# ricklisz/AnatoMask

Hardware: AMD Instinct MI355X
Metric: pretrain volumes/sec @128^3 patch mask=0.6 (higher is better)
Workload: dtype bf16; 1 GPU; STUNet-B AnatoMask step, 128^3 patch, mask_ratio 0.6, bf16 storage/MFMA + fp32 master; per_gpu_batch=16, global_batch=16, parallelism=dp1, step=teacher fwd + sampler + student fwd + loss + bwd + clip + AdamW + EMA

## Files before the change

### anatomask_amd/csrc/conv_igemm.hip

```cpp
#include <mutex>
#include <type_traits>
#include <stdlib.h>
#include "common.h"
#include "../../include/anatomask_hip.h"
#include "conv_plan.h"

using namespace amconv;

namespace {

template <typename T, int BD, int BH, int BW, int NS, int NIT, int TGS = 3, bool HR = false, bool NB = false, bool HT = false>
__global__ __launch_bounds__(256, (TGS == 2 && BD * BH * BW <= 256) ? 3 : 2) void conv_igemm_kernel(ConvArgs a) {
  constexpr int EPC = TT<T>::EPC;
  constexpr bool SPL = std::is_same<T, f32s_t>::value;
  constexpr int KC = (ROWB / 16) * EPC;
  constexpr int MV = BD * BH * BW;
  constexpr int VS = MV / 64;
  constexpr int NT = 16 * NS;
  constexpr int TG = TG_OF(NS, TGS);
  constexpr int WBUF = TG * NT * ROWB;
  constexpr int WCH = TG * NT * 4;
  constexpr int WIT = (WCH + 255) / 256;
  static_assert(MV % 64 == 0, "brick must give each wave whole 16-voxel subtiles");
  extern __shared__ __attribute__((aligned(16))) unsigned char lds[];
// ... 592 lines not shown
  p.in_sparse = p.out_sparse = sparse; p.same_mask = p.has_list = true;
  p.in_bshift = in_bshift; p.out_bshift = out_bshift; p.n_active = n_active;
}

extern "C" int am_conv3d_partials_rows(int mode, int dtype, int ksize, int stride, int B, int Do, int Ho, int Wo, int Cin, int Cout, int out_sparse,
                                       int out_bshift, int n_active, int* rows) {
  ConvProblem p{mode, dtype, ksize, stride, B, Do, Ho, Wo, Cin, Do, Ho, Wo, Cout};
  query_masks(p, out_sparse != 0, out_bshift, out_bshift, n_active);
  *rows = 0;
  for (const ConvStage& s : conv_stages) { const int r = s.fits(p); if (r > *rows) *rows = r; }
  return 0;
}

extern "C" int am_conv3d_uses_k3(int mode, int dtype, int ksize, int stride, int B, int Di, int Hi, int Wi, int Cin, int Do, int Ho, int Wo, int Cout,
                                 int has_masks, int accumulate, int fused_epilogue, int want_partials) {
  ConvProblem p{mode, dtype, ksize, stride, B, Di, Hi, Wi, Cin, Do, Ho, Wo, Cout};
  query_masks(p, has_masks != 0, 0, 0, 0);
  p.accumulate = accumulate != 0; p.ep = fused_epilogue != 0; p.partials = want_partials != 0;
  for (const ConvStage& s : conv_stages)
    if (s.serves(p)) return s.launch == conv_k3t_launch ? 2 : s.launch == conv_k3_launch ? 1 : 0;
  return 0;
}

static ConvArgs fill_args(const ConvProblem& p, const void* x, const void* w_packed, const float* bias, void* y, float* partials, const uint8_t* in_mask,
                          int in_bshift, const uint8_t* out_mask, int out_bshift, int fd, int fh, int fw, int accumulate) {
  ConvArgs a{};
  a.x = x; a.w = w_packed; a.bias = bias; a.y = y; a.partials = partials;
  a.B = p.B; a.Di = p.Di; a.Hi = p.Hi; a.Wi = p.Wi; a.Cin = p.Cin; a.Do = p.Do; a.Ho = p.Ho; a.Wo = p.Wo; a.Cout = p.Cout;
  am_packed_dims(p.dtype, p.Cout, p.Cin, &a.Coutp, &a.Cinp);
  a.w_bytes = p.ksize * p.ksize * p.ksize * a.Coutp * a.Cinp * (p.dtype == AM_DT_BF16 ? 2 : 4);
  a.in_mask = MaskView{in_mask, fd, fh, fw, in_bshift};
  a.out_mask = MaskView{out_mask, fd, fh, fw, out_bshift};
  a.accumulate = accumulate & 1; a.stats_sum_only = (accumulate & AM_CONV_PARTIALS_SUM_ONLY) ? 1 : 0;
#ifdef AM_ABLATE
  { const char* e = getenv("AM_CV_DBG"); a.dbg = e ? atoi(e) : 0; }
#endif
  return a;
}

static int conv3d_impl(ConvProblem& p, ConvArgs& a, const int* active_list, int n_active, void* stream, int* rows) {
  if (p.Cin % 8 || p.Cout % 8) return -1;
  p.in_sparse = a.in_mask.m != nullptr; p.out_sparse = a.out_mask.m != nullptr; p.same_mask = a.in_mask.m == a.out_mask.m;
  p.in_bshift = a.in_mask.bs; p.out_bshift = a.out_mask.bs; p.fd = a.in_mask.fd; p.fh = a.in_mask.fh; p.fw = a.in_mask.fw;
  p.has_list = active_list != nullptr; p.n_active = n_active;
  p.accumulate = a.accumulate != 0; p.sum_only = a.stats_sum_only != 0; p.partials = a.partials != nullptr;
  p.ep = a.ep_scale || a.ep_res || a.ep_act != AM_ACT_NONE; p.nbred = a.nb_x != nullptr; p.prenorm = a.in_scale != nullptr;
// ... 24 lines not shown
  query_masks(p, true, in_bshift, out_bshift, n_active);
  p.prenorm = true;
  return conv_rw_serves(p) ? 1 : 0;
}

extern "C" int am_conv3d_prenorm(int mode, int dtype, int ksize, int stride, const void* x, const void* w_packed, const float* bias, void* y,
                                 int B, int Di, int Hi, int Wi, int Cin, int Do, int Ho, int Wo, int Cout, const uint8_t* mask, int in_bshift,
                                 int out_bshift, int fd, int fh, int fw, float* partials, const float* in_scale, const float* in_shift,
                                 int in_act, const int32_t* active_list, int n_active, int* partial_rows_written, void* stream) {
  if (!in_scale || !in_shift || !mask || !active_list) return -1;
  if (in_act != AM_ACT_NONE && in_act != AM_ACT_LRELU && in_act != AM_ACT_RELU6) return -1;
  ConvProblem p{mode, dtype, ksize, stride, B, Di, Hi, Wi, Cin, Do, Ho, Wo, Cout};
  ConvArgs a = fill_args(p, x, w_packed, bias, y, partials, mask, in_bshift, mask, out_bshift, fd, fh, fw, 0);
  a.in_scale = in_scale; a.in_shift = in_shift; a.in_act = in_act;
  return conv3d_impl(p, a, active_list, n_active, stream, partial_rows_written);
}

extern "C" int am_conv3d_nbred(int mode, int dtype, int ksize, int stride, const void* x, const void* w_packed, void* y, int B, int Di,
                               int Hi, int Wi, int Cin, int Do, int Ho, int Wo, int Cout, const uint8_t* in_mask, int in_bshift,
                               const uint8_t* out_mask, int out_bshift, int fd, int fh, int fw, int accumulate, float* partials,
                               const void* nb_x, const float* nb_scale, const float* nb_shift, int nb_act,
                               int* partial_rows_written, void* stream) {
  if (dtype != AM_DT_BF16 || !partials || !nb_x) return -1;
  if (nb_act != AM_ACT_NONE && (!nb_scale || !nb_shift)) return -1;
  if (nb_act != AM_ACT_NONE && nb_act != AM_ACT_LRELU && nb_act != AM_ACT_RELU6) return -1;
  ConvProblem p{mode, dtype, ksize, stride, B, Di, Hi, Wi, Cin, Do, Ho, Wo, Cout};
  ConvArgs a = fill_args(p, x, w_packed, nullptr, y, partials, in_mask, in_bshift, out_mask, out_bshift, fd, fh, fw, accumulate);
  a.nb_x = nb_x; a.nb_scale = nb_scale; a.nb_shift = nb_shift; a.nb_act = nb_act;
  return conv3d_impl(p, a, nullptr, 0, stream, partial_rows_written);
}
```

### anatomask_amd/csrc/conv_k3.hip

```cpp
#include <stdlib.h>
#include "common.h"
#include "../../include/anatomask_hip.h"
#include "conv_plan.h"

using namespace amconv;

namespace {

constexpr int KBD = 8, KBH = 4, KBW = 16;
constexpr int KED = KBD + 2, KEH = KBH + 2, KEW = KBW + 2;
constexpr int KPLANE = KEH * KEW;
constexpr int KNROW = KED * KPLANE;
constexpr int KBRICKB = KNROW * 64;
constexpr int KNPIECE = 68;
constexpr int KWSLOT = 3 * 64 * 64;
constexpr int KLDS_W = 2 * KBRICKB;
constexpr int KLDS_TAB = KLDS_W + 2 * KWSLOT;
constexpr int KLDS = KLDS_TAB + 768;
#ifndef AM_K3_MIN_UNITS
#define AM_K3_MIN_UNITS 256
#endif
constexpr int K3_MIN_UNITS = AM_K3_MIN_UNITS;

struct K3Args {
// ... 5 lines not shown
  int nt_store;
  unsigned w_bytes;
#ifdef AM_ABLATE
  int dbg;
#endif
};

#define K3_LDSP(off) ((__attribute__((address_space(3))) void*)(lds + (off)))

__device__ __forceinline__ int k3_uni(int v) { return __builtin_amdgcn_readfirstlane(v); }
template <typename P> __device__ __forceinline__ P* k3_uni_ptr(P* p) {
  const unsigned long long v = (unsigned long long)p;
  const unsigned lo = (unsigned)__builtin_amdgcn_readfirstlane((int)(unsigned)v), hi = (unsigned)__builtin_amdgcn_readfirstlane((int)(unsigned)(v >> 32));
  return (P*)(((unsigned long long)hi << 32) | lo);
}

struct Item { int u, k, c0, c1, p; };
#define IT_Q0W(it) (((it).c0 & 255) * KBW)
#define IT_Q0H(it) ((((it).c0 >> 8) & 255) * KBH)
#define IT_Q0D(it) ((((it).c0 >> 16) & 255) * KBD)
#define IT_B(it) ((it).c1 & 255)
#define IT_CO0(it) (((it).c1 >> 8) * NT)

template <int NS, bool EP, bool ST, bool CT = false, bool S1 = false>
__global__ __launch_bounds__(512, 2) void conv_k3_kernel(K3Args a) {
  static_assert(NS == 4 || NS == 2, "64- or 32-channel output tiles (NS = 2: the decoder's last conv, C -> C / 2 = 32 at STUNet-B; a wave then owns 8 accumulator tiles)");
  constexpr int VS = 4, NT = 16 * NS;
  constexpr int NCH = VS * NS / 2;
  constexpr int NRUN = CT ? 4 : 9;
  constexpr int NTR = CT ? 2 : 3;
  static_assert(!CT || (NS == 4 && !EP && !ST), "transposed conv: 64-channel tiles, plain epilogue (bias)");
  static_assert(!S1 || (ST && NS == 4 && !CT), "sum-only statistics: a variant of the statistics instantiation");
  extern __shared__ __attribute__((aligned(16))) unsigned char lds[];
  const int tid = threadIdx.x, lane = tid & 63;
  const int wave = __builtin_amdgcn_readfirstlane(tid >> 6);
  const bool isX = wave < 4;
  const int wq = wave & 3;
  const int g = lane >> 4, r16 = lane & 15;
  const int G = gridDim.x;

  const int gperm = (G % 8 == 0) ? (int)(blockIdx.x % 8) * (G / 8) + (int)(blockIdx.x / 8) : (int)blockIdx.x;
  auto decode = [&](Item& it) {
    int br = it.u / a.ny;
    const int yt = it.u - br * a.ny;
    const int bw_ = br % a.nbw; br /= a.nbw;
    const int bh_ = br % a.nbh; br /= a.nbh;
    const int bd_ = br % a.nbd;
    it.c0 = k3_uni(bw_ | (bh_ << 8) | (bd_ << 16)); it.c1 = k3_uni((br / a.nbd) | (yt << 8));
  };
  auto advance = [&](Item& it) {
    if (it.k + 1 < a.nslab) { ++it.k; return; }
    it.k = 0;
    if (CT && it.p < 7) { ++it.p; return; }
    it.p = 0; it.u += G;
    if (it.u < a.nunit) decode(it);
// ... 48 lines not shown
    const long long org = ((((long long)IT_B(it) * a.D + (q0d - 1)) * a.H + (q0h - 1)) * a.W + (q0w - 1)) * (long long)a.Cin;
    const __amdgpu_buffer_rsrc_t rx = __builtin_amdgcn_make_buffer_rsrc((void*)k3_uni_ptr(a.x + org), 0, 0x7fffff00, 0x00020000);
#pragma unroll
    for (int k = k0; k < k1; ++k) {
      const unsigned bad = pbits[k / 5] & (m << (6 * (k % 5)));
      unsigned vo = bad ? OOB : pl[k];
#ifdef AM_ABLATE
      if (a.dbg & 2) vo = OOB;
#endif
      const int p = wave + 8 * k;
      const int row0 = p * 16 < KNROW - 16 ? p * 16 : KNROW - 16;
      __builtin_amdgcn_raw_ptr_buffer_load_lds(rx, K3_LDSP(sbuf * KBRICKB + row0 * 64), 16, vo, (unsigned)(it.k * 64), 0, 0);
    }
  };

  f32x4 acc[NS][VS];
  float f1[NS / 2][4], f2[NS / 2][4];
#pragma unroll
  for (int h = 0; h < NS / 2; ++h)
#pragma unroll
    for (int r = 0; r < 4; ++r) { f1[h][r] = 0.f; f2[h][r] = 0.f; }
  const unsigned oddm = (lane & 1) ? 0xffffffffu : 0u;
#ifdef AM_ABLATE
  const bool want_stats = ST && a.partials != nullptr && !(a.dbg & 32);
#else
  const bool want_stats = ST && a.partials != nullptr;
#endif
  bf16_t* __restrict__ yg = a.y;
  const float act_slope = a.ep_act == AM_ACT_LRELU ? 0.01f : (a.ep_act == AM_ACT_RELU6 ? 0.f : 1.f);
  const float act_hi = a.ep_act == AM_ACT_RELU6 ? 6.f : __builtin_inff();
  constexpr bool fused = EP;
  typedef __attribute__((ext_vector_type(4))) __bf16 bfx4;
  typedef __attribute__((ext_vector_type(8))) __bf16 bfx8;
  typedef __attribute__((ext_vector_type(8))) float f32x8;

  auto flush_stats = [&](const int co0) __attribute__((always_inline)) {
    float* part = a.partials + ((size_t)blockIdx.x * 8 + wave) * a.Cout * 2;
#define K3_DPP_ADD(V, CTRL) V += __builtin_bit_cast(float, __builtin_amdgcn_update_dpp(0, __builtin_bit_cast(int, V), CTRL, 0xF, 0xF, true))
#pragma unroll
    for (int h = 0; h < NS / 2; ++h)
#pragma unroll
      for (int r = 0; r < 4; ++r) {
        float s1 = f1[h][r], s2 = f2[h][r];
        K3_DPP_ADD(s1, 0x4E); K3_DPP_ADD(s1, 0x124); K3_DPP_ADD(s1, 0x128);
        if constexpr (!S1) { K3_DPP_ADD(s2, 0x4E); K3_DPP_ADD(s2, 0x124); K3_DPP_ADD(s2, 0x128); }
        const int c = co0 + h * 32 + g * 8 + (r16 & 1) * 4 + r;
        if (r16 < 2) { part[c * 2] = s1; part[c * 2 + 1] = s2; }
      }
#undef K3_DPP_ADD
// ... 86 lines not shown
  auto store_chunk = [&](const int c, const bool tail) __attribute__((always_inline)) {
    const int j = c / (NS / 2), h = c % (NS / 2);
    const __amdgpu_buffer_rsrc_t ry = __builtin_amdgcn_make_buffer_rsrc((void*)k3_uni_ptr(yg + pk_off), 0, 0x7fffff00, 0x00020000);
#ifdef AM_ABLATE
    if (!(a.dbg & 1))
#endif
    {
      u32x4 sv = pk[j][h];
      unsigned so_ = (unsigned)(j * orow + h * 64);
      if constexpr (FULL) {
        const u32x4 ot = pk[j][h ^ 1];
        u32x4 rx_;
#pragma unroll
        for (int e = 0; e < 4; ++e) rx_[e] = (unsigned)__builtin_amdgcn_update_dpp(0, (int)ot[e], 0x128, 0xF, 0xF, false);
        const bool own = h == 0 ? lo8 : !lo8;
#pragma unroll
        for (int e = 0; e < 4; ++e) sv[e] = own ? sv[e] : rx_[e];
        so_ = (unsigned)(j * orow) + (h ? ohalf : 0u);
      }
      if (a.nt_store) __builtin_amdgcn_raw_buffer_store_b128(sv, ry, olane, so_, 2);
      else __builtin_amdgcn_raw_buffer_store_b128(sv, ry, olane, so_, 0);
      if (tail || FULL) asm volatile("s_nop 4" : "+v"(sv) :: "memory");
    }
    if (want_stats && (tail || !spread_stats)) { stats_half(c, 0); stats_half(c, 1); }
  };

  if (want_stats && a.ny > 1) {
    float* part = a.partials + ((size_t)blockIdx.x * 8 + wave) * a.Cout * 2;
    for (int c = lane; c < a.Cout * 2; c += 64) part[c] = 0.f;
    asm volatile("s_waitcnt vmcnt(0)" ::: "memory");
  }
  if (tid < NT) {
    const int c = IT_CO0(cur) + tid;
    ((float*)(lds + KLDS_TAB))[tid] = a.bias ? a.bias[c] : 0.f;
    ((float*)(lds + KLDS_TAB))[64 + tid] = a.ep_scale ? a.ep_scale[c] : 1.f;
    ((float*)(lds + KLDS_TAB))[128 + tid] = a.ep_scale ? a.ep_shift[c] : 0.f;
  }
  if (isX) { issue_weights(cur, 0, 0); issue_pieces(cur, 0, 0, 9); }
  else issue_pieces(cur, 0, 0, 8);
  asm volatile("s_waitcnt vmcnt(0) lgkmcnt(0)" ::: "memory");
  __builtin_amdgcn_s_barrier();

#ifdef AM_ABLATE
  unsigned tL = 0, tWL = 0, tM = 0, tWM = 0, tE = 0, t_prev = 0;
  unsigned long long rt0 = 0;
  const bool stamps = (a.dbg & 16) != 0;
#define K3_STAMP(ACC) if (stamps) { unsigned long long t_; asm volatile("s_memtime %0\n\ts_waitcnt lgkmcnt(0)" : "=s"(t_) :: "memory"); ACC += (unsigned)t_ - t_prev; t_prev = (unsigned)t_; }
// ... 5 lines not shown
  int pc0 = 0, pc1 = 0, pcls = 0; bool have_prev = false;
  bool spend = false;
  bool pend_stats = false;
#pragma unroll
  for (int i = 0; i < NS; ++i)
#pragma unroll
    for (int j = 0; j < VS; ++j) acc[i][j] = f32x4{0.f, 0.f, 0.f, 0.f};
  while (true) {
    spend = false;
    if (cur.k == 0 && have_prev) {
      finish_unit(pc0, pc1, pcls);
      spend = true; pend_stats = true;
      K3_STAMP(tE);
    } else if (cur.k >= 2) pend_stats = false;
    const bool has_next = nxt.u < a.nunit;
    int bxc[3];
#pragma unroll
    for (int xw = 0; xw < 3; ++xw) bxc[xw] = bx[xw] + sb * KBRICKB;
    const bool fetch_next = has_next && (!CT || a.nslab != 2 || nxt.p == 0);
    const int cpd = (cur.p >> 2) & 1, cph = (cur.p >> 1) & 1, cpw = cur.p & 1;
#pragma unroll
    for (int run = 0; run < NRUN; ++run) {
      const int zd = run / 3, xw = run % 3;
      u32x4 brow[VS + 2], af[3][NS];
      const int wbase = KLDS_W + par * KWSLOT + aoff;
      if constexpr (CT) {
        const int zq = cpd + (run >> 1), xq = cpw + (run & 1);
        const int bsel = (xq == 0 ? bxc[0] : (xq == 1 ? bxc[1] : bxc[2])) + (zq * KPLANE + cph * KEW) * 64;
#pragma unroll
        for (int r = 0; r < VS + 1; ++r) brow[r] = *(const u32x4*)(lds + bsel + r * KEW * 64);
      } else {
#pragma unroll
      for (int r = 0; r < VS + 2; ++r) brow[r] = *(const u32x4*)(lds + bxc[xw] + (zd * KPLANE + r * KEW) * 64);
      }
#pragma unroll
      for (int th = 0; th < NTR; ++th)
#pragma unroll
        for (int i = 0; i < NS; ++i) af[th][i] = *(const u32x4*)(lds + wbase + th * (NT * 64) + i * 1024);
      const int pk0 = CT ? (isX ? 3 * run : 4 * run) : (run == 0 ? 0 : (run == 1 ? 1 : run + 1));
      const int npx = CT ? (run < 3 ? 3 : 0) : (run == 1 ? 2 : (run < 8 ? 1 : 0));
      const int npy = CT ? (run < 2 ? 4 : 0) : (run == 1 ? 2 : (run < 7 ? 1 : 0));
      constexpr int SPR = CT ? 2 : 1;
      if (isX) {
        if (run < NRUN - 1) issue_weights(cur, run + 1, par ^ 1);
        else if (has_next) issue_weights(nxt, 0, par ^ 1);
        if (fetch_next && npx > 0) issue_pieces(nxt, sb ^ 1, CT ? 3 * run : pk0, (CT ? 3 * run : pk0) + npx);
// ... 38 lines not shown
        else if (nbehind == 2) asm volatile("s_waitcnt vmcnt(2)" ::: "memory");
        else if (nbehind == 3) asm volatile("s_waitcnt vmcnt(3)" ::: "memory");
        else if (nbehind == 4) asm volatile("s_waitcnt vmcnt(4)" ::: "memory");
        else asm volatile("s_waitcnt vmcnt(5)" ::: "memory");
      } else if (run == NRUN - 2) {
        if (spend && run * SPR < NCH) { if (SPR == 2) asm volatile("s_waitcnt vmcnt(2)" ::: "memory"); else asm volatile("s_waitcnt vmcnt(1)" ::: "memory"); }
        else asm volatile("s_waitcnt vmcnt(0)" ::: "memory");
      }
      K3_STAMP(tM);
      if (isX) {
        __builtin_amdgcn_s_barrier();
        K3_STAMP(tWM);
      }
      par ^= 1;
    }
    sb ^= 1;
    if (cur.k + 1 == a.nslab) { pc0 = cur.c0; pc1 = cur.c1; pcls = cur.p; have_prev = true; }
    if (!has_next) break;
    cur = nxt; advance(nxt);
  }
  finish_unit(pc0, pc1, pcls);
#pragma unroll
  for (int c = 0; c < NCH; ++c) store_chunk(c, true);
  if (want_stats) flush_stats((pc1 >> 8) * NT);
#ifdef AM_ABLATE
  if (stamps && a.partials) {
    K3_STAMP(tE);
    unsigned long long rt1; asm volatile("s_memrealtime %0\n\ts_waitcnt lgkmcnt(0)" : "=s"(rt1) :: "memory");
    unsigned* row = (unsigned*)(a.partials + ((size_t)blockIdx.x * 8 + wave) * a.Cout * 2);
    asm volatile("s_waitcnt vmcnt(0)" ::: "memory");
    if (lane == 0) { row[0] = tL; row[1] = tWL; row[2] = tM; row[3] = tWM; row[4] = tE; row[5] = (unsigned)(rt1 - rt0); }
  }
#endif
}

}

namespace amconv {

static int k3_tiles(int Cout) { return Cout % 64 ? Cout / 32 : Cout / 64; }
static int k3_units(int B, int D, int H, int W, int Cout) { return B * (D / KBD) * (H / KBH) * (W / KBW) * k3_tiles(Cout); }
static int k3_grid(int units, int Cout, int dev = am_device()) {
  const int cus = am_cu_count(dev), ny = k3_tiles(Cout);
  const int G = units < cus ? units : cus;
  return G - G % ny > 0 ? G - G % ny : ny;
}

static bool k3_qualifies(int mode, int dtype, int ksize, int stride, int B, int D, int H, int W, int Cin, int Cout, bool masks) {
  if (dtype != AM_DT_BF16 || ksize != 3 || stride != 1 || (mode != AM_CONV_FWD && mode != AM_CONV_DGRAD) || masks) return false;
  if (Cin % 32 || Cout % 32 || D % KBD || H % KBH || W % KBW) return false;
  if (B > 255 || D / KBD > 255 || H / KBH > 255 || W / KBW > 255) return false;
  return k3_units(B, D, H, W, Cout) >= K3_MIN_UNITS;
}

int conv_k3_fits(const ConvProblem& p) {
  if (!k3_qualifies(p.mode, p.dtype, p.ksize, p.stride, p.B, p.Do, p.Ho, p.Wo, p.Cin, p.Cout, p.in_sparse || p.out_sparse)) return 0;
  return k3_grid(k3_units(p.B, p.Do, p.Ho, p.Wo, p.Cout), p.Cout) * 8;
}

bool conv_k3_serves(const ConvProblem& p) {
#ifdef AM_ABLATE
  if (getenv("AM_CV_NORW") || getenv("AM_CV_NOK3")) return false;
  { const char* e_ = getenv("AM_K3_NO32"); if (e_ && atoi(e_) && p.Cout % 64) return false; }
#endif
  if (!conv_k3_fits(p) || p.prenorm || p.accumulate || p.nbred) return false;
  if (p.Di != p.Do || p.Hi != p.Ho || p.Wi != p.Wo) return false;
  if ((size_t)(KED + 1) * p.Hi * p.Wi * p.Cin * 2 >= 0x7fffff00ull) return false;
  if (p.ep && p.partials) return false;
  return true;
}

int conv_k3t_fits(const ConvProblem&) { return 0; }
bool conv_k3t_serves(const ConvProblem& p) {
#ifdef AM_ABLATE
  if (getenv("AM_CV_NORW")) return false;
  { const char* e_ = getenv("AM_CV_NOK3T"); if (e_ && atoi(e_)) return false; }
#endif
  if (p.mode != AM_CONVT_FWD || p.dtype != AM_DT_BF16 || p.ksize != 4 || p.stride != 2 || p.in_sparse || p.out_sparse) return false;
  if (p.prenorm || p.accumulate || p.nbred || p.partials || p.ep) return false;
  if (p.Cin % 32 || p.Cin < 64 || p.Cout % 64 || p.Di % KBD || p.Hi % KBH || p.Wi % KBW) return false;
  if (p.Do != 2 * p.Di || p.Ho != 2 * p.Hi || p.Wo != 2 * p.Wi) return false;
  if (p.B > 255 || p.Di / KBD > 255 || p.Hi / KBH > 255 || p.Wi / KBW > 255) return false;
  if ((size_t)(KED + 1) * p.Hi * p.Wi * p.Cin * 2 >= 0x7fffff00ull || (size_t)16 * p.Wo * p.Cout * 2 >= 0x7fffff00ull) return false;
  return k3_units(p.B, p.Di, p.Hi, p.Wi, p.Cout) >= K3_MIN_UNITS;
}

static void k3_fill(K3Args& a, const ConvProblem& p, const ConvArgs& c) {
  a.x = (const bf16_t*)c.x; a.w = (const bf16_t*)c.w; a.bias = c.bias; a.y = (bf16_t*)c.y; a.partials = c.partials;
  a.ep_scale = c.ep_scale; a.ep_shift = c.ep_shift; a.ep_res = (const bf16_t*)c.ep_res; a.ep_act = c.ep_act;
  a.B = c.B; a.D = c.Di; a.H = c.Hi; a.W = c.Wi; a.Cin = c.Cin; a.Cout = c.Cout; a.Cinp = c.Cinp; a.Coutp = c.Coutp;
  a.nbd = c.Di / KBD; a.nbh = c.Hi / KBH; a.nbw = c.Wi / KBW; a.ny = k3_tiles(c.Cout); a.nunit = k3_units(c.B, c.Di, c.Hi, c.Wi, c.Cout); a.nslab = c.Cinp / 32;
  a.flip = p.mode == AM_CONV_DGRAD;
  a.nt_store = (size_t)c.B * c.Do * c.Ho * c.Wo * c.Cout * 2 >= ((size_t)384 << 20);
  a.w_bytes = (unsigned)c.w_bytes;
#ifdef AM_ABLATE
  { const char* e = getenv("AM_K3_DBG"); a.dbg = e ? atoi(e) : 0; }
#endif
}

int conv_k3_launch(const ConvProblem& p, ConvArgs& c, const int*, void* stream, int* rows) {
  if (!conv_k3_serves(p)) return 0;
  const int dev = am_device();
  K3Args a;
  k3_fill(a, p, c);
  const int G = k3_grid(a.nunit, c.Cout, dev);
  auto kern = p.ep ? conv_k3_kernel<4, true, false> : (a.partials ? conv_k3_kernel<4, false, true> : conv_k3_kernel<4, false, false>);
  if (c.Cout % 64) kern = p.ep ? conv_k3_kernel<2, true, false> : (a.partials ? conv_k3_kernel<2, false, true> : conv_k3_kernel<2, false, false>);
  else if (a.partials && !p.ep && c.stats_sum_only) kern = conv_k3_kernel<4, false, true, false, true>;
  AM_HIP_STAGE((am_lds_optin<conv_k3_kernel<4, true, false>, conv_k3_kernel<4, false, true>, conv_k3_kernel<4, false, false>,
                             conv_k3_kernel<2, true, false>, conv_k3_kernel<2, false, true>, conv_k3_kernel<2, false, false>,
                             conv_k3_kernel<4, false, true, false, true>>(dev)));
  AM_LAUNCH(kern, dim3(G), dim3(512), KLDS, (hipStream_t)stream, a);
  AM_CHECK_LAUNCH_STAGE();
  if (rows) *rows = G * 8;
  return 1;
}

int conv_k3t_launch(const ConvProblem& p, ConvArgs& c, const int*, void* stream, int*) {
  if (!conv_k3t_serves(p)) return 0;
  const int dev = am_device();
  K3Args a;
  k3_fill(a, p, c);
  constexpr auto kern = conv_k3_kernel<4, false, false, true>;
  AM_HIP_STAGE(am_lds_optin<kern>(dev));
  AM_LAUNCH(kern, dim3(k3_grid(a.nunit, c.Cout, dev)), dim3(512), KLDS, (hipStream_t)stream, a);
  AM_CHECK_LAUNCH_STAGE();
  return 1;
}

}
```

### anatomask_amd/csrc/conv_plan.h

```cpp
#pragma once
#include "common.h"

namespace amconv {

struct ConvArgs {
  const void* x; const void* w; const float* bias; void* y; float* partials;
  const float* ep_scale; const float* ep_shift; const void* ep_res; int ep_act;
  const void* nb_x; const float* nb_scale; const float* nb_shift; int nb_act;
  const float* in_scale; const float* in_shift; int in_act;
  int B, Di, Hi, Wi, Cin, Do, Ho, Wo, Cout, Cinp, Coutp;
  int OS, GS, nclass, nunit;
  int ny;
  int nbd, nbh, nbw;
  int tap_begin[9];
  int upar[8];
  int taps[64];
  int mind[8], minh[8], minw[8];
  int ed[8], eh[8], ew[8];
  int mdiv_w[8], mdiv_hw[8];
  int w_bytes;
  int w_lds_off;
  MaskView in_mask, out_mask;
  int accumulate;
  int stats_sum_only;
// ... 81 lines not shown
  return 0;
}


struct ConvProblem {
  int mode, dtype, ksize, stride, B, Di, Hi, Wi, Cin, Do, Ho, Wo, Cout;
  bool in_sparse, out_sparse, same_mask, has_list;
  int in_bshift, out_bshift, n_active, fd, fh, fw;
  bool accumulate, ep, partials, sum_only;
  bool nbred, prenorm;
};

struct ConvStage {
  const char* name;
  int (*fits)(const ConvProblem&);
  bool (*serves)(const ConvProblem&);
  int (*launch)(const ConvProblem&, ConvArgs& a, const int* active_list, void* stream, int* rows);
};
#define AM_CONV_STAGE(name_) int name_##_fits(const ConvProblem&); bool name_##_serves(const ConvProblem&); \
                             int name_##_launch(const ConvProblem&, ConvArgs&, const int*, void*, int*)
AM_CONV_STAGE(conv_k3t); AM_CONV_STAGE(conv_k3);
AM_CONV_STAGE(conv_rw); AM_CONV_STAGE(conv_gather);
AM_CONV_STAGE(conv_igemm);

}
```

### anatomask_amd/engine.py

```python
from __future__ import annotations

from dataclasses import dataclass, field
from typing import Dict, List, Optional, Sequence, Tuple

import torch

from . import ops
from .ops import ACT_LRELU, ACT_NONE, ACT_RELU6, CONV_DGRAD, CONV_FWD, CONVT_DGRAD, CONVT_FWD, MaskInfo, NormStats

ENC = "sparse_encoder.sp_cnn.conv_blocks_context"
DEC = "dense_decoder.dec"


@dataclass
class Spec:
    dims: Sequence[int]
    depth: Sequence[int]
    width: int
    input_size: Tuple[int, int, int]
    in_ch: int = 1
    out_ch: int = 1
    downsample: int = 16
    n_stage: int = 5
    sync_bn: bool = False
# ... 392 lines not shown
    def run():
        dwp = ops.conv3d_wgrad(mode, x, dy, k, stride, f32_split=pk.f32_split, deterministic=pk.deterministic, **masks)
        ops.unpack_grad(dwp, G[name], transposed, accumulate=True)
    _on_side(x.device, (x, dy), run)


def _dec_block_backward(W, G, pk: PackCache, t: dict, g: Optional[torch.Tensor], drec: Optional[torch.Tensor], bias_sum_into: Optional[torch.Tensor]):
    q = t["q"]
    if t.get("inorm"):
        so = tuple(t["r"].shape[1:4])
        dc2 = _instance_norm_backward(g, t["c2"], t["st2"], ACT_NONE)
        dr = ops.conv3d(CONV_DGRAD, dc2, pk.get(W, f"{q}.conv.3.weight", False, True), None, so, 3, 1)
        _wgrad_into(pk, G, f"{q}.conv.3.weight", CONV_FWD, t["r"], dc2, 3, 1)
        dc1 = _instance_norm_backward(dr, t["c1"], t["st1"], ACT_RELU6)
    elif t.get("head"):
        dc2 = ops.proj_norm_bwd(t["c2"], t["st2"], drec, W["dense_decoder.proj.weight"].view(-1), W[f"{q}.conv.4.weight"],
                                W[f"{q}.conv.4.bias"], G[f"{q}.conv.4.weight"], G[f"{q}.conv.4.bias"],
                                G["dense_decoder.proj.weight"].view(-1), G["dense_decoder.proj.bias"])
    else:
        dc2 = ops.norm_backward(g, None, t["c2"], t["st2"], W[f"{q}.conv.4.weight"], ACT_NONE, None, 0,
                                G[f"{q}.conv.4.weight"], G[f"{q}.conv.4.bias"])
    if not t.get("inorm"):
        so = tuple(t["r"].shape[1:4])
        fuse = ops.FUSED_NORM_BWD_REDUCE and dc2.dtype == torch.bfloat16 and t["st1"].sync_world <= 1 and dc2.shape[-1] >= 128
        dr = ops.conv3d(CONV_DGRAD, dc2, pk.get(W, f"{q}.conv.3.weight", False, True), None, so, 3, 1,
                        norm_bwd=(t["c1"], t["st1"], ACT_RELU6) if fuse else None)
        dr, red1 = dr if fuse else (dr, None)
        _wgrad_into(pk, G, f"{q}.conv.3.weight", CONV_FWD, t["r"], dc2, 3, 1)
        dc1 = ops.norm_backward(dr, None, t["c1"], t["st1"], W[f"{q}.conv.1.weight"], ACT_RELU6, None, 0,
                                G[f"{q}.conv.1.weight"], G[f"{q}.conv.1.bias"], reduced=red1)
    du, ptu = ops.conv3d(CONV_DGRAD, dc1, pk.get(W, f"{q}.conv.0.weight", False, True), None, so, 3, 1, want_partials=True, partials_sum_only=True)
    ptu.finalize(None, sum_accum=G[f"{q}.up_sample.bias"])
    _wgrad_into(pk, G, f"{q}.conv.0.weight", CONV_FWD, t["u"], dc1, 3, 1)
    si = tuple(t["xin"].shape[1:4])
    gin = ops.conv3d(CONVT_DGRAD, du, pk.get(W, f"{q}.up_sample.weight", True, True), None, si, 4, 2, want_partials=bias_sum_into is not None)
    if bias_sum_into is not None:
        gin, ptg = gin
        ptg.finalize(None, sum_accum=bias_sum_into)
    _wgrad_into(pk, G, f"{q}.up_sample.weight", CONVT_FWD, t["xin"], du, 4, 2, transposed=True)
    return gin


def decoder_backward(spec: Spec, W, G, pk: PackCache, tape: Tape, drec: torch.Tensor, after_group=None) -> List[Optional[torch.Tensor]]:
    n_dec = len(spec.dec_chs) - 1
    fused_head = bool(tape.dec[n_dec - 1].get("head"))
    g = None
    if not fused_head:
        g = ops.proj_bwd(tape.last, drec, W["dense_decoder.proj.weight"].view(-1), G["dense_decoder.proj.weight"].view(-1),
# ... 174 lines not shown
```

### anatomask_amd/hip.py

```python
import ctypes as C
import os
import re

_HERE = os.path.dirname(os.path.abspath(__file__))
LIB_PATH = os.path.join(_HERE, "libanatomask_hip.so")
HEADER = os.path.join(os.path.dirname(_HERE), "include", "anatomask_hip.h")

DT_F32, DT_BF16, DT_F32S = 0, 1, 2
CONV_FWD, CONV_DGRAD, CONVT_FWD, CONVT_DGRAD = 0, 1, 2, 3
ACT_NONE, ACT_LRELU, ACT_RELU6 = 0, 1, 2

_CT = {"int": C.c_int, "long": C.c_long, "float": C.c_float, "double": C.c_double}


def declared_functions(header: str = HEADER):
    txt = open(header).read()
    txt = re.sub(r"/\*.*?\*/", " ", txt, flags=re.S)
    out = {}
    for m in re.finditer(r"\bint\s+(am_\w+)\s*\(([^;]*?)\)\s*;", txt, flags=re.S):
        name, args = m.group(1), m.group(2).strip()
        types = []
        if args and args != "void":
            for a in args.split(","):
                a = " ".join(a.split())
                if "*" in a:
                    types.append(C.c_void_p)
                else:
                    types.append(_CT[a.replace("const ", "").split(" ")[0]])
        out[name] = types
    return out


class HipLib:
    ANSWERS = ("am_head_stencil_supported", "am_conv3d_wgrad_uses_k3", "am_conv3d_uses_k3", "am_conv3d_prenorm_supported", "am_version")

    def __init__(self, path: str = LIB_PATH):
        import torch
        if not os.path.exists(path):
            raise RuntimeError(f"{path} not built: run `python -m anatomask_amd.build` (no fallback path exists)")
        if os.path.abspath(path) == LIB_PATH:
            from . import build as _b
            sp = _b.stamp_path(path)
            have = open(sp).read().strip() if os.path.exists(sp) else None
            if have != _b.source_digest():
                raise RuntimeError(f"{path} was not built from the csrc/ + include/ sources next to it (stamp {str(have)[:12]}.. != sources "
                                   f"{_b.source_digest()[:12]}..): run `python -m anatomask_amd.build`")
        self._lib = C.CDLL(path)
        self.functions = declared_functions()
        for name, argtypes in self.functions.items():
            fn = getattr(self._lib, name)
            fn.argtypes = argtypes
            fn.restype = C.c_int
            if name not in self.ANSWERS:
                setattr(self, name[3:], self._wrap(name, fn))

    @staticmethod
    def _wrap(name, fn):
# ... 25 lines not shown
```

### anatomask_amd/ops.py

```python
from __future__ import annotations

from typing import Optional, Tuple

import torch

from . import hip
from .hip import ACT_LRELU, ACT_NONE, ACT_RELU6, CONV_DGRAD, CONV_FWD, CONVT_DGRAD, CONVT_FWD


def _dt(t: torch.Tensor) -> int:
    if t.dtype == torch.float32:
        return hip.DT_F32
    if t.dtype == torch.bfloat16:
        return hip.DT_BF16
    raise TypeError(f"unsupported dtype {t.dtype}")


DEFAULT_F32_SPLIT = False


def _dtc(t: torch.Tensor, f32_split: bool) -> int:
    return hip.DT_F32S if (t.dtype == torch.float32 and f32_split) else _dt(t)


# ... 429 lines not shown
        ws_b[:NREP * Cc * 3].zero_()
        if dx is None:
            dx = torch.empty_like(x)
        L.norm_bwd_apply(_dt(x), dout.data_ptr(), _p(out), x.data_ptr(), B, D, H, W, Cc, mp, bshift, fd, fh, fw,
                         st.mean.data_ptr(), st.rstd.data_ptr(), sc.k[0].data_ptr(), sc.k[1].data_ptr(), sc.k[2].data_ptr(), act,
                         dx.data_ptr(), _p(dres), _p(dxsum), ws_x.data_ptr(), st.scale.data_ptr(), st.shift.data_ptr(), *_al(mask), 0, s)
        if dxsum is not None:
            ws_x[:DXREP * Cc].zero_()
        return dx
    L.norm_bwd_reduce(_dt(x), dout.data_ptr(), _p(out), x.data_ptr(), B, D, H, W, Cc, mp, bshift, fd, fh, fw,
                      st.mean.data_ptr(), st.rstd.data_ptr(), act, int(fill), ws_b.data_ptr(), st.scale.data_ptr(), st.shift.data_ptr(),
                      *_al(mask), _p(st.count_ptr), float(st.count_host), gamma.data_ptr(), sc.k[0].data_ptr(), sc.k[1].data_ptr(),
                      sc.k[2].data_ptr(), _p(dgamma), _p(dbeta), _p(dtoken), _p(dbeta2), s)
    if dx is None:
        dx = torch.empty_like(x)
    L.norm_bwd_apply(_dt(x), dout.data_ptr(), _p(out), x.data_ptr(), B, D, H, W, Cc, mp, bshift, fd, fh, fw,
                     st.mean.data_ptr(), st.rstd.data_ptr(), sc.k[0].data_ptr(), sc.k[1].data_ptr(), sc.k[2].data_ptr(), act,
                     dx.data_ptr(), _p(dres), _p(dxsum), ws_x.data_ptr(), st.scale.data_ptr(), st.shift.data_ptr(), *_al(mask), 1, s)
    return dx


_BWS = {}
FUSED_BWD_TAILS = True
FUSED_NORM_BWD_REDUCE = False


def _bwd_workspaces(device, C: int):
    key = (device, torch.cuda.current_stream(device).cuda_stream)
    ws = _BWS.get(key)
    if ws is None or ws[2] < C:
        cap = max(C, 2048)
        ws = _BWS[key] = (torch.zeros(NREP * cap * 3 + 2, device=device, dtype=torch.float64),
                          torch.zeros(DXREP * cap + 2, device=device, dtype=torch.float64), cap)
    return ws[0], ws[1]


def chan_sum(x: torch.Tensor, mask: Optional[MaskInfo], bshift: int, out_accum: torch.Tensor):
    B, D, H, W, Cc = x.shape
    mp, fd, fh, fw = _mk(mask)
    hip.lib().chan_sum(_dt(x), x.data_ptr(), B, D, H, W, Cc, mp, bshift, fd, fh, fw, out_accum.data_ptr(), _stream())


def add(a: torch.Tensor, b: torch.Tensor, out: Optional[torch.Tensor] = None) -> torch.Tensor:
    if out is None:
        out = torch.empty_like(a)
    hip.lib().add(_dt(a), a.data_ptr(), b.data_ptr(), out.data_ptr(), a.numel(), _stream())
    return out
# ... 226 lines not shown
```

### include/anatomask_hip.h

```cpp
#ifndef ANATOMASK_HIP_H
#define ANATOMASK_HIP_H
#include <stdint.h>
#ifdef __cplusplus
extern "C" {
#endif

#define AM_DT_F32 0
#define AM_DT_BF16 1
#define AM_DT_F32S 2

#define AM_CONV_PARTIALS_SUM_ONLY 2
#define AM_CONV_FWD 0
#define AM_CONV_DGRAD 1
#define AM_CONVT_FWD 2
#define AM_CONVT_DGRAD 3

#define AM_DXREP 64
#define AM_NREP 8

#define AM_ACT_NONE 0
#define AM_ACT_LRELU 1
#define AM_ACT_RELU6 2

int am_version(void);

int am_conv3d(int mode, int dtype, int ksize, int stride, const void* x, const void* w_packed, const float* bias, void* y,
              int B, int Di, int Hi, int Wi, int Cin, int Do, int Ho, int Wo, int Cout,
              const uint8_t* in_mask, int in_bshift, const uint8_t* out_mask, int out_bshift, int fd, int fh, int fw,
              int accumulate, float* partials ,
              const float* ep_scale, const float* ep_shift ,
              const void* ep_res ,
              int ep_act ,
              const int32_t* active_list, int n_active ,
              int* partial_rows_written ,
              void* stream);
int am_conv3d_prenorm_supported(int mode, int dtype, int ksize, int stride, int B, int Do, int Ho, int Wo, int Cin, int Cout, int sparse,
                                int in_bshift, int out_bshift, int n_active);
int am_conv3d_prenorm(int mode, int dtype, int ksize, int stride, const void* x, const void* w_packed, const float* bias, void* y, int B, int Di,
                      int Hi, int Wi, int Cin, int Do, int Ho, int Wo, int Cout, const uint8_t* mask, int in_bshift, int out_bshift, int fd,
                      int fh, int fw, float* partials , const float* in_scale, const float* in_shift, int in_act,
                      const int32_t* active_list, int n_active, int* partial_rows_written , void* stream);

int am_conv3d_nbred(int mode, int dtype, int ksize, int stride, const void* x, const void* w_packed, void* y, int B, int Di,
                    int Hi, int Wi, int Cin, int Do, int Ho, int Wo, int Cout, const uint8_t* in_mask, int in_bshift,
                    const uint8_t* out_mask, int out_bshift, int fd, int fh, int fw, int accumulate, float* partials,
                    const void* nb_x, const float* nb_scale, const float* nb_shift, int nb_act,
                    int* partial_rows_written, void* stream);
int am_packed_dims(int dtype, int rows, int k, int* rows_padded, int* k_padded);
int am_conv3d_partials_rows(int mode, int dtype, int ksize, int stride, int B, int Do, int Ho, int Wo, int Cin, int Cout,
                            int out_sparse, int out_bshift ,
                            int n_active, int* rows );
int am_conv3d_uses_k3(int mode, int dtype, int ksize, int stride, int B, int Di, int Hi, int Wi, int Cin, int Do, int Ho, int Wo, int Cout,
                      int has_masks, int accumulate, int fused_epilogue, int want_partials);
int am_partials_reduce(const float* partials, int rows, int C, double* sums, float* sum_accum, void* stream);

int am_conv3d_wgrad(int mode, int dtype, int ksize, int stride, const void* x, const void* dy, float* dw_packed,
                    int B, int Dx, int Hx, int Wx, int Cx, int Dy, int Hy, int Wy, int Cy,
                    const uint8_t* x_mask, int x_bshift, const uint8_t* y_mask, int y_bshift, int fd, int fh, int fw,
                    float* det_workspace, long det_workspace_floats,
                    const int32_t* active_list, int n_active ,
                    void* gather_workspace, long gather_workspace_bytes ,
                    void* stream);
int am_conv3d_wgrad_uses_k3(int mode, int dtype, int ksize, int stride, int B, int D, int H, int W, int Cx, int Cy, int has_masks,
                            int deterministic);
int am_conv3d_wgrad_gather_bytes(int mode, int dtype, int ksize, int stride, int B, int Cx, int Cy, int y_bshift, int has_y_mask, int n_active,
                                 int fd, int fh, int fw, long* bytes );

int am_split_bf16(const float* x, void* hi, void* lo, long n, void* stream);

int am_pack_weight(int dtype, const float* src, void* dst, int R, int K, int taps, long stride_r, long stride_k, int Rp, int Kp,
// ... 159 lines not shown
```

Baseline: 139.1 volumes/s.

## Fuse norm-backward reduction into k3 dgrad conv kernel and enable by default

Adds an NB instantiation of the k3 3x3x3 conv kernel that, while computing the dgrad output, reloads the saved activation, applies the ReLU6 mask from the norm scale/shift, and accumulates per-channel sum(g) and sum(g*x) partials. The loads are overlapped with the conv's run loop. A query entry point lets the engine decide per layer whether the k3 path serves and pays off (Cin >= 64). The fused norm-backward reduce is turned on by default, which also drops the old channel >= 128 restriction. This removes a separate reduction pass over the gradient and activation. The cost is extra register and VMEM pressure inside a hand-scheduled kernel whose waitcnt values are tuned by hand.

Result: no change. 140.5 volumes/s (median of 6 runs) (+1.0%).

```diff
diff --git a/anatomask_amd/csrc/conv_igemm.hip b/anatomask_amd/csrc/conv_igemm.hip
--- a/anatomask_amd/csrc/conv_igemm.hip
+++ b/anatomask_amd/csrc/conv_igemm.hip
@@ -638,6 +638,17 @@
   return 0;
 }
 
+extern "C" int am_conv3d_nbred_uses_k3(int mode, int dtype, int ksize, int stride, int B, int Di, int Hi, int Wi, int Cin, int Do, int Ho, int Wo,
+                                       int Cout, int has_masks, int accumulate) {
+  if (dtype != AM_DT_BF16 || (accumulate & ~1)) return 0;
+  ConvProblem p{mode, dtype, ksize, stride, B, Di, Hi, Wi, Cin, Do, Ho, Wo, Cout};
+  query_masks(p, has_masks != 0, 0, 0, 0);
+  p.accumulate = accumulate != 0; p.partials = true; p.nbred = true;
+  for (const ConvStage& s : conv_stages)
+    if (s.serves(p)) return s.launch == conv_k3_launch ? (conv_k3_nbred_pays(p) ? 1 : 2) : 0;
+  return 0;
+}
+
 static ConvArgs fill_args(const ConvProblem& p, const void* x, const void* w_packed, const float* bias, void* y, float* partials, const uint8_t* in_mask,
                           int in_bshift, const uint8_t* out_mask, int out_bshift, int fd, int fh, int fw, int accumulate) {
   ConvArgs a{};
@@ -708,6 +719,7 @@
                                const void* nb_x, const float* nb_scale, const float* nb_shift, int nb_act,
                                int* partial_rows_written, void* stream) {
   if (dtype != AM_DT_BF16 || !partials || !nb_x) return -1;
+  if (accumulate & ~1) return -1;
   if (nb_act != AM_ACT_NONE && (!nb_scale || !nb_shift)) return -1;
   if (nb_act != AM_ACT_NONE && nb_act != AM_ACT_LRELU && nb_act != AM_ACT_RELU6) return -1;
   ConvProblem p{mode, dtype, ksize, stride, B, Di, Hi, Wi, Cin, Do, Ho, Wo, Cout};
diff --git a/anatomask_amd/csrc/conv_k3.hip b/anatomask_amd/csrc/conv_k3.hip
--- a/anatomask_amd/csrc/conv_k3.hip
+++ b/anatomask_amd/csrc/conv_k3.hip
@@ -51,7 +51,7 @@
 #define IT_B(it) ((it).c1 & 255)
 #define IT_CO0(it) (((it).c1 >> 8) * NT)
 
-template <int NS, bool EP, bool ST, bool CT = false, bool S1 = false>
+template <int NS, bool EP, bool ST, bool CT = false, bool S1 = false, bool NB = false>
 __global__ __launch_bounds__(512, 2) void conv_k3_kernel(K3Args a) {
   static_assert(NS == 4 || NS == 2, "64- or 32-channel output tiles (NS = 2: the decoder's last conv, C -> C / 2 = 32 at STUNet-B; a wave then owns 8 accumulator tiles)");
   constexpr int VS = 4, NT = 16 * NS;
@@ -60,6 +60,7 @@
   constexpr int NTR = CT ? 2 : 3;
   static_assert(!CT || (NS == 4 && !EP && !ST), "transposed conv: 64-channel tiles, plain epilogue (bias)");
   static_assert(!S1 || (ST && NS == 4 && !CT), "sum-only statistics: a variant of the statistics instantiation");
+  static_assert(!NB || (NS == 4 && !EP && !ST && !CT), "norm-backward reduce: a variant of the plain 64-channel instantiation");
   extern __shared__ __attribute__((aligned(16))) unsigned char lds[];
   const int tid = threadIdx.x, lane = tid & 63;
   const int wave = __builtin_amdgcn_readfirstlane(tid >> 6);
@@ -154,9 +155,9 @@
     for (int r = 0; r < 4; ++r) { f1[h][r] = 0.f; f2[h][r] = 0.f; }
   const unsigned oddm = (lane & 1) ? 0xffffffffu : 0u;
 #ifdef AM_ABLATE
-  const bool want_stats = ST && a.partials != nullptr && !(a.dbg & 32);
+  const bool want_stats = (ST || NB) && a.partials != nullptr && !(a.dbg & 32);
 #else
-  const bool want_stats = ST && a.partials != nullptr;
+  const bool want_stats = (ST || NB) && a.partials != nullptr;
 #endif
   bf16_t* __restrict__ yg = a.y;
   const float act_slope = a.ep_act == AM_ACT_LRELU ? 0.01f : (a.ep_act == AM_ACT_RELU6 ? 0.f : 1.f);
@@ -289,7 +290,72 @@
       else __builtin_amdgcn_raw_buffer_store_b128(sv, ry, olane, so_, 0);
       if (tail || FULL) asm volatile("s_nop 4" : "+v"(sv) :: "memory");
     }
-    if (want_stats && (tail || !spread_stats)) { stats_half(c, 0); stats_half(c, 1); }
+    if (ST && want_stats && (tail || !spread_stats)) { stats_half(c, 0); stats_half(c, 1); }
+  };
+  const unsigned nb_so[2] = {0u, ohalf};
+  auto nb_stored = [&](const int c) __attribute__((always_inline)) {
+    const int j = c / (NS / 2), h = c % (NS / 2);
+    u32x4 sv = pk[j][h];
+    const u32x4 ot = pk[j][h ^ 1];
+    const bool own = h == 0 ? lo8 : !lo8;
+#pragma unroll
+    for (int e = 0; e < 4; ++e) {
+      const unsigned rx_ = (unsigned)__builtin_amdgcn_update_dpp(0, (int)ot[e], 0x128, 0xF, 0xF, false);
+      sv[e] = own ? sv[e] : rx_;
+    }
+    return sv;
+  };
+  auto nb_load = [&](const int c) __attribute__((always_inline)) {
+    const int j = c / (NS / 2), h = c % (NS / 2);
+    const __amdgpu_buffer_rsrc_t rr = __builtin_amdgcn_make_buffer_rsrc((void*)k3_uni_ptr(a.ep_res + pk_off), 0, 0x7fffff00, 0x00020000);
+    return (u32x4)__builtin_amdgcn_raw_buffer_load_b128(rr, olane, (unsigned)(j * orow) + nb_so[h], 0);
+  };
+  const int nbtab = KLDS_TAB + 256 + ((r16 >> 3) * 32 + g * 8) * 4;
+  auto nb_stats = [&](const int c, const u32x4 xv) __attribute__((always_inline)) {
+    const u32x4 gv = nb_stored(c);
+    const bool has_act = a.ep_act != AM_ACT_NONE;
+#pragma unroll
+    for (int q = 0; q < 2; ++q) {
+      f32x4 sc = {1.f, 1.f, 1.f, 1.f}, sh = {0.f, 0.f, 0.f, 0.f};
+      if (has_act) { sc = *(const f32x4*)(lds + nbtab + q * 16); sh = *(const f32x4*)(lds + nbtab + 256 + q * 16); }
+#pragma unroll
+      for (int r = 0; r < 4; ++r) {
+        const unsigned gw = gv[2 * q + (r >> 1)], xw = xv[2 * q + (r >> 1)];
+        float gf = __uint_as_float((r & 1) ? (gw & 0xffff0000u) : (gw << 16));
+        const float xf = __uint_as_float((r & 1) ? (xw & 0xffff0000u) : (xw << 16));
+        if (has_act) {
+          const float z = xf * sc[r] + sh[r];
+          gf *= (z > 0.f && z < act_hi) ? 1.f : act_slope;
+        }
+        f1[q][r] += gf;
+        f2[q][r] += gf * xf;
+      }
+    }
+  };
+  auto nb_flush = [&](const int co0) __attribute__((always_inline)) {
+    float* part = a.partials + ((size_t)blockIdx.x * 8 + wave) * a.Cout * 2;
+#define K3_DPP_ADD(V, CTRL) V += __builtin_bit_cast(float, __builtin_amdgcn_update_dpp(0, __builtin_bit_cast(int, V), CTRL, 0xF, 0xF, true))
+#pragma unroll
+    for (int q = 0; q < 2; ++q)
+#pragma unroll
+      for (int r = 0; r < 4; ++r) {
+        float s1 = f1[q][r], s2 = f2[q][r];
+        K3_DPP_ADD(s1, 0xB1); K3_DPP_ADD(s1, 0x4E); K3_DPP_ADD(s1, 0x141);
+        K3_DPP_ADD(s2, 0xB1); K3_DPP_ADD(s2, 0x4E); K3_DPP_ADD(s2, 0x141);
+        const int c = co0 + (r16 >> 3) * 32 + g * 8 + q * 4 + r;
+        if ((r16 & 7) == 0) { part[c * 2] = s1; part[c * 2 + 1] = s2; }
+      }
+#undef K3_DPP_ADD
+  };
+  u32x4 nbq = {0u, 0u, 0u, 0u};
+  auto nb_issue = [&](const int c) __attribute__((always_inline)) {
+    const int j = c / (NS / 2), h = c % (NS / 2);
+    const unsigned long long pa = (unsigned long long)(a.ep_res + pk_off);
+    u32x4 rs;
+    rs[0] = (unsigned)__builtin_amdgcn_readfirstlane((int)(unsigned)pa); rs[1] = (unsigned)__builtin_amdgcn_readfirstlane((int)(unsigned)(pa >> 32)) & 0xffffu;
+    rs[2] = 0x7fffff00u; rs[3] = 0x00020000u;
+    const int so_ = k3_uni((int)((unsigned)(j * orow) + nb_so[h]));
+    asm volatile("s_nop 4\n\tbuffer_load_dwordx4 %0, %1, %2, %3 offen" : "=v"(nbq) : "v"(olane), "s"(rs), "s"(so_) : "memory");
   };
 
   if (want_stats && a.ny > 1) {
@@ -341,6 +407,19 @@
 #pragma unroll
     for (int run = 0; run < NRUN; ++run) {
       const int zd = run / 3, xw = run % 3;
+      if constexpr (NB) {
+        if (spend && want_stats && run >= 1 && run <= NCH) {
+          if (!isX) {
+            const int q_ = run - 1, young = 1 + (fetch_next ? (q_ == 1 ? 2 : (q_ < 7 ? 1 : 0)) : 0);
+            if (young == 1) asm volatile("s_waitcnt vmcnt(1)" ::: "memory");
+            else if (young == 2) asm volatile("s_waitcnt vmcnt(2)" ::: "memory");
+            else asm volatile("s_waitcnt vmcnt(3)" ::: "memory");
+          }
+          __builtin_amdgcn_sched_barrier(0);
+          nb_stats(run - 1, nbq);
+        }
+        if (spend && want_stats && run < NCH) nb_issue(run);
+      }
       u32x4 brow[VS + 2], af[3][NS];
       const int wbase = KLDS_W + par * KWSLOT + aoff;
       if constexpr (CT) {
@@ -425,7 +504,13 @@
   finish_unit(pc0, pc1, pcls);
 #pragma unroll
   for (int c = 0; c < NCH; ++c) store_chunk(c, true);
-  if (want_stats) flush_stats((pc1 >> 8) * NT);
+  if constexpr (NB) {
+    if (want_stats) {
+#pragma unroll
+      for (int c = 0; c < NCH; ++c) { nbq = nb_load(c); nb_stats(c, nbq); }
+    }
+  }
+  if (want_stats) { if constexpr (NB) nb_flush((pc1 >> 8) * NT); else flush_stats((pc1 >> 8) * NT); }
 #ifdef AM_ABLATE
   if (stamps && a.partials) {
     K3_STAMP(tE);
@@ -466,12 +551,15 @@
   if (getenv("AM_CV_NORW") || getenv("AM_CV_NOK3")) return false;
   { const char* e_ = getenv("AM_K3_NO32"); if (e_ && atoi(e_) && p.Cout % 64) return false; }
 #endif
-  if (!conv_k3_fits(p) || p.prenorm || p.accumulate || p.nbred) return false;
+  if (!conv_k3_fits(p) || p.prenorm || p.accumulate) return false;
+  if (p.nbred && (p.Cout % 64 || !p.partials || p.sum_only || p.ep)) return false;
   if (p.Di != p.Do || p.Hi != p.Ho || p.Wi != p.Wo) return false;
   if ((size_t)(KED + 1) * p.Hi * p.Wi * p.Cin * 2 >= 0x7fffff00ull) return false;
   if (p.ep && p.partials) return false;
   return true;
 }
+
+bool conv_k3_nbred_pays(const ConvProblem& p) { return p.Cin >= 64; }
 
 int conv_k3t_fits(const ConvProblem&) { return 0; }
 bool conv_k3t_serves(const ConvProblem& p) {
@@ -510,9 +598,13 @@
   auto kern = p.ep ? conv_k3_kernel<4, true, false> : (a.partials ? conv_k3_kernel<4, false, true> : conv_k3_kernel<4, false, false>);
   if (c.Cout % 64) kern = p.ep ? conv_k3_kernel<2, true, false> : (a.partials ? conv_k3_kernel<2, false, true> : conv_k3_kernel<2, false, false>);
   else if (a.partials && !p.ep && c.stats_sum_only) kern = conv_k3_kernel<4, false, true, false, true>;
+  if (p.nbred) {
+    kern = conv_k3_kernel<4, false, false, false, false, true>;
+    a.ep_res = (const bf16_t*)c.nb_x; a.ep_scale = c.nb_scale; a.ep_shift = c.nb_scale ? c.nb_shift : nullptr; a.ep_act = c.nb_act;
+  }
   AM_HIP_STAGE((am_lds_optin<conv_k3_kernel<4, true, false>, conv_k3_kernel<4, false, true>, conv_k3_kernel<4, false, false>,
                              conv_k3_kernel<2, true, false>, conv_k3_kernel<2, false, true>, conv_k3_kernel<2, false, false>,
-                             conv_k3_kernel<4, false, true, false, true>>(dev)));
+                             conv_k3_kernel<4, false, true, false, true>, conv_k3_kernel<4, false, false, false, false, true>>(dev)));
   AM_LAUNCH(kern, dim3(G), dim3(512), KLDS, (hipStream_t)stream, a);
   AM_CHECK_LAUNCH_STAGE();
   if (rows) *rows = G * 8;
diff --git a/anatomask_amd/csrc/conv_plan.h b/anatomask_amd/csrc/conv_plan.h
--- a/anatomask_amd/csrc/conv_plan.h
+++ b/anatomask_amd/csrc/conv_plan.h
@@ -127,5 +127,6 @@
 AM_CONV_STAGE(conv_k3t); AM_CONV_STAGE(conv_k3);
 AM_CONV_STAGE(conv_rw); AM_CONV_STAGE(conv_gather);
 AM_CONV_STAGE(conv_igemm);
+bool conv_k3_nbred_pays(const ConvProblem&);
 
 }
diff --git a/anatomask_amd/engine.py b/anatomask_amd/engine.py
--- a/anatomask_amd/engine.py
+++ b/anatomask_amd/engine.py
@@ -438,8 +438,12 @@
                                 G[f"{q}.conv.4.weight"], G[f"{q}.conv.4.bias"])
     if not t.get("inorm"):
         so = tuple(t["r"].shape[1:4])
-        fuse = ops.FUSED_NORM_BWD_REDUCE and dc2.dtype == torch.bfloat16 and t["st1"].sync_world <= 1 and dc2.shape[-1] >= 128
-        dr = ops.conv3d(CONV_DGRAD, dc2, pk.get(W, f"{q}.conv.3.weight", False, True), None, so, 3, 1,
+        wd3 = pk.get(W, f"{q}.conv.3.weight", False, True)
+        fuse = bool(ops.FUSED_NORM_BWD_REDUCE) and dc2.dtype == torch.bfloat16 and t["st1"].sync_world <= 1
+        if fuse:
+            k3 = ops.conv3d_nbred_uses_k3(CONV_DGRAD, dc2, wd3, so, 3, 1)
+            fuse = k3 == 1 or (k3 == 2 and int(ops.FUSED_NORM_BWD_REDUCE) >= 2)
+        dr = ops.conv3d(CONV_DGRAD, dc2, wd3, None, so, 3, 1,
                         norm_bwd=(t["c1"], t["st1"], ACT_RELU6) if fuse else None)
         dr, red1 = dr if fuse else (dr, None)
         _wgrad_into(pk, G, f"{q}.conv.3.weight", CONV_FWD, t["r"], dc2, 3, 1)
diff --git a/anatomask_amd/hip.py b/anatomask_amd/hip.py
--- a/anatomask_amd/hip.py
+++ b/anatomask_amd/hip.py
@@ -32,7 +32,7 @@
 
 
 class HipLib:
-    ANSWERS = ("am_head_stencil_supported", "am_conv3d_wgrad_uses_k3", "am_conv3d_uses_k3", "am_conv3d_prenorm_supported", "am_version")
+    ANSWERS = ("am_head_stencil_supported", "am_conv3d_wgrad_uses_k3", "am_conv3d_uses_k3", "am_conv3d_nbred_uses_k3", "am_conv3d_prenorm_supported", "am_version")
 
     def __init__(self, path: str = LIB_PATH):
         import torch
diff --git a/anatomask_amd/ops.py b/anatomask_amd/ops.py
--- a/anatomask_amd/ops.py
+++ b/anatomask_amd/ops.py
@@ -475,7 +475,14 @@
 
 _BWS = {}
 FUSED_BWD_TAILS = True
-FUSED_NORM_BWD_REDUCE = False
+FUSED_NORM_BWD_REDUCE = 1
+
+
+def conv3d_nbred_uses_k3(mode: int, x: torch.Tensor, w_packed: torch.Tensor, out_spatial, ksize: int, stride: int) -> int:
+    if x.dtype != torch.bfloat16 or w_packed.dtype != torch.bfloat16:
+        return 0
+    B, Di, Hi, Wi, Cin = x.shape
+    return hip.lib()._lib.am_conv3d_nbred_uses_k3(mode, _dt(x), ksize, stride, B, Di, Hi, Wi, Cin, *out_spatial, w_packed.logical[0], 0, 0)
 
 
 def _bwd_workspaces(device, C: int):
diff --git a/include/anatomask_hip.h b/include/anatomask_hip.h
--- a/include/anatomask_hip.h
+++ b/include/anatomask_hip.h
@@ -46,6 +46,8 @@
                     const uint8_t* out_mask, int out_bshift, int fd, int fh, int fw, int accumulate, float* partials,
                     const void* nb_x, const float* nb_scale, const float* nb_shift, int nb_act,
                     int* partial_rows_written, void* stream);
+int am_conv3d_nbred_uses_k3(int mode, int dtype, int ksize, int stride, int B, int Di, int Hi, int Wi, int Cin, int Do, int Ho, int Wo, int Cout,
+                            int has_masks, int accumulate);
 int am_packed_dims(int dtype, int rows, int k, int* rows_padded, int* k_padded);
 int am_conv3d_partials_rows(int mode, int dtype, int ksize, int stride, int B, int Do, int Ho, int Wo, int Cin, int Cout,
                             int out_sparse, int out_bshift ,
```
